# AtomGradient/swift-qwen3-tts

Hardware: AMD Instinct MI355X
Metric: codec_tokens_per_s (higher is better)
Workload: dtype bf16

## Files before the change

### include/q3tts.h

```cpp
#ifndef Q3TTS_H
#define Q3TTS_H

#include <stddef.h>
#include <stdint.h>

#ifdef __cplusplus
extern "C" {
#endif

#define Q3TTS_ABI_VERSION 4

typedef struct q3tts_model q3tts_model;

typedef enum {
    Q3TTS_OK = 0,
    Q3TTS_ERR_MODEL_NOT_INITIALIZED = 1,
    Q3TTS_ERR_GENERATION_FAILED = 2,
    Q3TTS_ERR_INVALID_INPUT = 3,
    Q3TTS_ERR_AUDIO_DECODING_FAILED = 4,
    Q3TTS_ERR_AUDIO_ENCODING_FAILED = 5,
    Q3TTS_ERR_IO = 6,
    Q3TTS_ERR_DEVICE = 7,
    Q3TTS_ERR_CANCELLED = 8,
    Q3TTS_ERR_BUSY = 9
// ... 287 lines not shown
    const uint8_t* active;
    const int32_t* block_table;
    const int32_t* chunk_n_prompt;
    uint16_t* kpool;
    uint16_t* vpool;
    uint16_t* out;
} q3tts_attn_debug;
q3tts_status q3tts_debug_attention(q3tts_model* m, const q3tts_attn_debug* a);

typedef struct {
    int32_t mode, geometry_only;
    int32_t M, K, N;
    int32_t xMB, yMB, ss_ld, y_cols;
    int32_t epi, act_silu, resid, nt_weights, y_tiled;
    int32_t norm, quant, has_bias;
    int32_t ss_count, norm_dim;
    float norm_eps;
    int32_t rider_M, rider_H, rider_MB, rider_ss_count;
    float rider_eps;
    int32_t rode;
    int32_t tall;
    int32_t tall_shape;
    int32_t split, mbw, nw, ch, np, gx, ntw;
    const uint16_t* x;
    const void* W;
    const uint16_t* scales;
    const uint16_t* biases;
    const void* W_up;
    const uint16_t* scales_up;
    const uint16_t* biases_up;
    const uint16_t* bias;
    const uint16_t* norm_w;
    const float* ss_in;
    const uint16_t* rider_h;
    const uint16_t* rider_w;
    const float* rider_ss_in;
    uint16_t* y;
    float* ss_out;
    uint16_t* rider_out;
    float* rider_ss_out;
} q3tts_gemm_debug;
q3tts_status q3tts_debug_gemm(q3tts_model* m, q3tts_gemm_debug* a);

typedef struct {
    int32_t kind, geometry_only, split;
    int32_t B, Tmax, ppf, hist, margin;
// ... 73 lines not shown
```

### swift-qwen3-tts_amd/csrc/debug_env.cc

```cpp
#include <atomic>
#include <cstdlib>
#include <mutex>

#include "kernels.h"

namespace q3 {

namespace {
std::mutex g_mu;
std::atomic<const DebugEnv*> g_env{nullptr};

bool flag(const char* name) { return std::getenv(name) != nullptr; }
int number(const char* name, int dflt) {
    const char* e = std::getenv(name);
    return e && *e ? std::atoi(e) : dflt;
}

const DebugEnv* read_env() {
    DebugEnv* d = new DebugEnv{};
    d->gemm_no_row_split = flag("Q3TTS_GEMM_NO_ROW_SPLIT");
    d->gemm_one_pair = flag("Q3TTS_GEMM_ONE_PAIR");
    d->no_tall_gemm = flag("Q3TTS_NO_TALL_GEMM");
    d->tall_shape = number("Q3TTS_TALL_SHAPE", 0);
    d->chunk_qsplit = number("Q3TTS_CHUNK_QSPLIT", 0);
    d->conv_no_pw = flag("Q3TTS_CONV_NO_PW");
    d->nt_off = std::getenv("Q3TTS_NT") && number("Q3TTS_NT", 1) == 0;
    d->serial_jobs = number("Q3TTS_SERIAL_JOBS", 0) != 0;
    d->fail_back_half = number("Q3TTS_TEST_FAIL_BACK_HALF", 0) != 0;
    d->no_prefix_cache = number("Q3TTS_NO_PREFIX_CACHE", 0) != 0;
    return d;
}
}

const DebugEnv& debug_env() {
    const DebugEnv* e = g_env.load(std::memory_order_acquire);
    if (!e) {
        std::lock_guard<std::mutex> lk(g_mu);
        e = g_env.load(std::memory_order_acquire);
        if (!e) {
            e = read_env();
            g_env.store(e, std::memory_order_release);
        }
    }
    return *e;
// ... 9 lines not shown
```

### swift-qwen3-tts_amd/csrc/engine_debug.cc

```cpp
#include "engine_stream.h"

#include "frontend.h"

namespace q3 {

void Engine::debug_frontend_stage(const float* audio, int64_t n_samples, const char* stage, float* out, int64_t cap, int* T, int* C) {
    Q3_CHECK(fe_ != nullptr, 1, "Model not initialized: Speech tokenizer encoder not available");
    Q3_CHECK(audio && n_samples > 0 && stage, 3, "Invalid input: empty audio or stage name");
    const float* a = upload_audio(audio, n_samples);
    StageCapture cap_s;
    cap_s.name = stage;
    static const char* kSpeaker[] = {"mel", "h0", "h1", "h2", "h3", "mfa", "pooled"};
    bool is_spk = false;
    for (const char* s : kSpeaker) is_spk = is_spk || cap_s.name == s;
    if (is_spk) {
        Q3_CHECK(m_->has_speaker_encoder, 1, "Model not initialized: Speaker encoder not available for this model");
        spk_f32_.grow(size_t(m_->cfg.talker.hidden_size));
        fe_->speaker_embedding(a, n_samples, spk_f32_, &cap_s);
    } else {
        Q3_CHECK(m_->has_codec_encoder, 1, "Model not initialized: Speech tokenizer encoder not available");
        const int Tq = fe_->encoded_frames(n_samples);
        ref_codes_dev_.grow(size_t(16) * Tq);
        fe_->encode(a, n_samples, ref_codes_dev_, &cap_s);
    }
// ... 262 lines not shown
    Q3_HIP(hipMemset(ot, 0xff, size_t(Mp) * odim * 2));
    AttnArgs at{};
    at.qkv = qkv; at.ld = ld; at.qn_w = w; at.kn_w = w + kHeadDim; at.eps = d.eps;
    at.rope_cos = rope; at.rope_sin = rope + tab;
    at.kpool = kp; at.vpool = vp;
    at.block_table = bt; at.max_pages = d.max_pages; at.kv_len = kv_len; at.active = d.active ? (const uint8_t*)act : nullptr;
    at.out = ot; at.outMB = Mp / 16; at.n_heads = d.n_heads; at.n_kv = d.n_kv; at.B = B;
    at.scale = d.scale;
    at.fixed_len = d.fixed_len; at.identity_pages = d.identity_pages ? 1 : 0;
    at.chunk = d.chunk; at.chunk_n_prompt = d.chunk_n_prompt ? n_prompt : nullptr; at.chunk_r_base = d.chunk_r_base;
    at.nt_kv = d.nt_kv ? 1 : 0;
    launch_attn_decode(at, st_);
    Q3_HIP(hipGetLastError());
    launch_untile_rows(ot, Mp / 16, ol, odim, rows, odim, st_);
    Q3_HIP(hipStreamSynchronize(st_));
    Q3_HIP(hipMemcpy(d.out, ol, size_t(rows) * odim * 2, hipMemcpyDeviceToHost));
    Q3_HIP(hipMemcpy(d.kpool, kp, pool * 2, hipMemcpyDeviceToHost));
    Q3_HIP(hipMemcpy(d.vpool, vp, pool * 2, hipMemcpyDeviceToHost));
}

void Engine::debug_gemm_check(q3tts_gemm_debug& d, GemmArgs& ga, NormRowsArgs& na) {
    static const uint16_t dummy16 = 0;
    static const uint32_t dummy32 = 0;
    d.rode = d.tall = d.tall_shape = d.split = d.mbw = d.nw = d.ch = d.np = d.gx = d.ntw = 0;
    Q3_CHECK(d.mode == 0 || d.mode == 1, 3, "debug_gemm: unknown mode");
    const bool rider = d.mode == 1 || d.rider_M > 0;
    if (rider) {
        Q3_CHECK(d.rider_M >= 1 && d.rider_MB >= 1 && d.rider_MB <= 64 && d.rider_M <= 16 * d.rider_MB, 3, "debug_gemm: rider rows out of range");
        Q3_CHECK(d.rider_H >= 128 && d.rider_H <= 4096 && d.rider_H % 128 == 0, 3, "debug_gemm: rider_H must be a multiple of 128 up to 4096");
        Q3_CHECK(d.geometry_only || (d.rider_h && d.rider_w && d.rider_out), 3, "debug_gemm: null rider argument");
        if (d.rider_ss_in) Q3_CHECK(d.rider_ss_count >= 1 && d.rider_ss_count <= 256, 3, "debug_gemm: at most 256 partial sums of squares per rider row");
        na.hMB = na.outMB = d.rider_MB; na.eps = d.rider_eps; na.M = d.rider_M; na.H = d.rider_H;
        na.ss_count = d.rider_ss_in ? d.rider_ss_count : 0; na.ss_ld = 16 * d.rider_MB;
    }
    if (d.mode == 1) return;
    Q3_CHECK(d.epi == 0 || d.epi == 2 || d.epi == 3, 3, "debug_gemm: unknown epilogue");
    Q3_CHECK(d.M >= 1 && d.M <= 1024, 3, "debug_gemm: M out of range");
    Q3_CHECK(d.K >= 128 && d.K <= 8192 && d.K % 128 == 0, 3, "debug_gemm: K must be a multiple of 128 up to 8192");
    Q3_CHECK(d.N >= 8 && d.N <= 65536 && d.N % (d.epi == 2 ? 8 : 16) == 0, 3, "debug_gemm: N must be a multiple of 16 (epi 2: of 8)");
    const int Mp = int(align_up(size_t(d.M), 16));
    const bool tiled = d.epi != 0 || d.y_tiled;
    Q3_CHECK(d.xMB <= 64 && 16 * d.xMB >= Mp && d.yMB <= 64 && 16 * d.yMB >= Mp && d.ss_ld >= Mp && d.ss_ld <= 4096, 3,
             "debug_gemm: allocation smaller than the padded batch");
    Q3_CHECK(d.y_cols >= d.N && d.y_cols <= d.N + 1024 && d.y_cols % (tiled ? 128 : 8) == 0, 3, "debug_gemm: y_cols");
    Q3_CHECK(d.epi != 2 || (!d.has_bias && !d.act_silu), 3, "debug_gemm: the gate/up epilogue takes no bias or activation");
    Q3_CHECK(d.epi == 0 || !d.act_silu, 3, "debug_gemm: act_silu belongs to epi 0");
    Q3_CHECK(d.epi == 3 || (!d.resid && !d.ss_out), 3, "debug_gemm: resid / ss_out belong to epi 3");
    if (d.norm) Q3_CHECK(d.ss_count >= 1 && d.ss_count <= 4096 && d.norm_dim >= 1, 3, "debug_gemm: norm prologue sizes");
    if (!d.geometry_only) {
        Q3_CHECK(d.x && d.W && d.y, 3, "debug_gemm: null argument");
        Q3_CHECK((d.epi == 2) == (d.W_up != nullptr), 3, "debug_gemm: W_up goes with epi 2");
        Q3_CHECK((d.quant != 0) == (d.scales != nullptr) && (d.quant != 0) == (d.biases != nullptr), 3, "debug_gemm: scales / biases go with quant");
        if (d.epi == 2) Q3_CHECK((d.quant != 0) == (d.scales_up != nullptr) && (d.quant != 0) == (d.biases_up != nullptr), 3, "debug_gemm: scales / biases go with quant");
        Q3_CHECK((d.has_bias != 0) == (d.bias != nullptr), 3, "debug_gemm: bias goes with has_bias");
        Q3_CHECK((d.norm != 0) == (d.norm_w != nullptr) && (d.norm != 0) == (d.ss_in != nullptr), 3, "debug_gemm: norm_w / ss_in go with norm");
    }
    ga.Wsb = d.quant ? &dummy32 : nullptr;
    ga.xMB = d.xMB; ga.M = d.M; ga.Mpad = Mp; ga.N = d.N; ga.K = d.K; ga.epi = d.epi;
    ga.ldy = d.y_cols; ga.y_tiled = d.y_tiled ? 1 : 0; ga.yMB = d.yMB;
    ga.bias = d.has_bias ? &dummy16 : nullptr;
    ga.act_silu = d.act_silu ? 1 : 0;
    ga.norm_w = d.norm ? &dummy16 : nullptr;
    ga.ss_count = d.norm ? d.ss_count : 0; ga.ss_ld = d.ss_ld; ga.norm_dim = d.norm_dim; ga.norm_eps = d.norm_eps;
    ga.nt_weights = d.nt_weights ? 1 : 0; ga.resid = d.resid ? 1 : 0;
    const SkinnyGeom g = skinny_geometry(ga);
    d.tall = g.tall ? 1 : 0;
    if (g.tall) {
        d.tall_shape = gemm_tall_shape(ga);
    } else {
        Q3_CHECK(g.mbw >= 1 && g.mbw <= 4, 3, "debug_gemm: more than 4 row blocks per workgroup");
        d.split = g.split; d.mbw = g.mbw; d.nw = g.nw; d.ch = g.ch; d.np = g.np; d.gx = g.gx; d.ntw = g.ntw ? 1 : 0;
    }
    if (rider) d.rode = gemm_norm_rows_rides(ga, na) ? 1 : 0;
}

namespace {
void host_tile(const uint16_t* src, std::vector<uint16_t>& dst, int rows, int cols) {
    dst.resize(size_t(rows) * cols);
    for (int m = 0; m < rows; ++m)
        for (int k = 0; k < cols; k += 8) std::memcpy(&dst[act_tiled_offset(m, k, rows / 16)], src + size_t(m) * cols + k, 16);
}
void host_untile(const std::vector<uint16_t>& src, uint16_t* dst, int rows, int cols) {
    for (int m = 0; m < rows; ++m)
        for (int k = 0; k < cols; k += 8) std::memcpy(dst + size_t(m) * cols + k, &src[act_tiled_offset(m, k, rows / 16)], 16);
}
}

void Engine::debug_gemm(q3tts_gemm_debug& d) {
    GemmArgs ga{};
    NormRowsArgs na{};
    debug_gemm_check(d, ga, na);
    DevBuf<uint16_t> dx, dy, dbias, dnw, dsrc, dsc, dbi, rh, rw, rout;
    DevBuf<uint8_t> dWt;
    DevBuf<uint32_t> dWq, dsb;
// ... 321 lines not shown
```

### swift-qwen3-tts_amd/csrc/kernels.h

```cpp
#pragma once
#include <hip/hip_runtime.h>

#include <cstdint>

namespace q3 {

struct DebugEnv {
    bool gemm_no_row_split;
    bool gemm_one_pair;
    bool no_tall_gemm;
    int tall_shape;
    int chunk_qsplit;
    bool conv_no_pw;
    bool nt_off;
    bool serial_jobs;
    bool fail_back_half;
    bool no_prefix_cache;
};
const DebugEnv& debug_env();
void debug_env_reload();

constexpr int kPageTokens = 64;
constexpr int kHeadDim = 128;

struct NormRowsArgs {
    const uint16_t* h;
    int hMB;
    const uint16_t* w;
    float eps;
    uint16_t* out;
    int outMB;
    float* ss_out;
// ... 10 lines not shown
    int xMB;
    int M, Mpad, N, K;
    int epi;
    uint16_t* y;
    int ldy;
    int y_tiled, yMB;
    const uint16_t* bias;
    int act_silu;
    const uint16_t* norm_w;
    const float* ss_in;
    int ss_count, ss_ld, norm_dim;
    float norm_eps;
    int nt_weights;
    int resid;
    float* ss_out;
};
void launch_gemm_skinny(const GemmArgs& a, hipStream_t st);
struct SkinnyGeom {
    bool tall;
    int split, mbw;
    int nw, ch, np;
    int gx;
    bool ntw;
};
SkinnyGeom skinny_geometry(const GemmArgs& a);
bool launch_gemm_skinny_with_norm_rows(const GemmArgs& a, const NormRowsArgs& n, hipStream_t st);
bool gemm_norm_rows_rides(const GemmArgs& a, const NormRowsArgs& n);
bool launch_gemm_tall(const GemmArgs& a, hipStream_t st);
bool gemm_tall_takes(const GemmArgs& a);
int gemm_tall_shape(const GemmArgs& a);


struct AttnArgs {
    const uint16_t* qkv;
    int ld;
    const uint16_t* qn_w;
    const uint16_t* kn_w;
    float eps;
    const uint16_t* rope_cos;
    const uint16_t* rope_sin;
    uint16_t* kpool;
    uint16_t* vpool;
    const int32_t* block_table;
    int max_pages;
    const int32_t* kv_len;
    const uint8_t* active;
// ... 166 lines not shown
```

### swift-qwen3-tts_amd/csrc/kernels/gemm_body.inc

```
__device__ __forceinline__ f32x4 mfma16(const uint4& a, const uint4& b, f32x4 c) {
    bf16x8 av, bv;
    __builtin_memcpy(&av, &a, 16);
    __builtin_memcpy(&bv, &b, 16);
    return __builtin_amdgcn_mfma_f32_16x16x32_bf16(av, bv, c, 0, 0, 0);
}

__device__ __forceinline__ float silu_f(float v) { return v / (1.0f + __expf(-v)); }

__device__ __forceinline__ uint4 norm8(const uint4& hx, const uint4& wx, float rstd) {
    const uint32_t hw[4] = {hx.x, hx.y, hx.z, hx.w}, ww[4] = {wx.x, wx.y, wx.z, wx.w};
    uint32_t o[4];
#pragma unroll
    for (int j = 0; j < 4; ++j) {
        const float n0 = rbf(lo_bf(hw[j]) * rstd), n1 = rbf(hi_bf(hw[j]) * rstd);
        o[j] = pack_bf(n0 * lo_bf(ww[j]), n1 * hi_bf(ww[j]));
    }
    return make_uint4(o[0], o[1], o[2], o[3]);
}

__device__ __forceinline__ void dequant_chunk(const uint4& qw, uint32_t sb, uint4 (&out)[4]) {
    const float sc = lo_bf(sb), bi = hi_bf(sb);
    const uint32_t w[4] = {qw.x, qw.y, qw.z, qw.w};
#pragma unroll
    for (int i = 0; i < 4; ++i) {
        uint32_t o[4];
#pragma unroll
        for (int j = 0; j < 4; ++j) {
            const float q0 = (float)((w[i] >> (8 * j)) & 15u), q1 = (float)((w[i] >> (8 * j + 4)) & 15u);
            o[j] = pack_bf(__fadd_rn(__fmul_rn(q0, sc), bi), __fadd_rn(__fmul_rn(q1, sc), bi));
        }
        out[i] = make_uint4(o[0], o[1], o[2], o[3]);
    }
}

template <int MB, int EPI, int NW, int CH, bool NORM, bool QUANT, int NP = 1, bool NTW = false>
__device__ __forceinline__ void gemm_skinny_body(const GemmArgs& a, const int tile, const int mb0) {
    constexpr int NT = NP;
    constexpr int NR = 1;
    const int n_tiles = (EPI == 2) ? (a.N >> 3) : (a.N >> 4);
    __shared__ float red[NW][NR][MB][4][64];
    __shared__ __attribute__((aligned(16))) uint16_t ys[MB][16][16];
    __shared__ float rstd_s[NORM ? 16 * MB : 1];
    __shared__ float ssp_s[NORM ? 8 : 1][NORM ? 16 * MB : 1];

    const int lane = threadIdx.x & 63;
    const int wave = threadIdx.x >> 6;
    const int KC = a.K >> 7;

    f32x4 acc[NT][MB];
#pragma unroll
    for (int t = 0; t < NT; ++t)
#pragma unroll
        for (int mb = 0; mb < MB; ++mb) acc[t][mb] = f32x4{0.f, 0.f, 0.f, 0.f};

    const uint4* Wt = reinterpret_cast<const uint4*>(a.W);
    const uint4* Xt = reinterpret_cast<const uint4*>(a.x);

    constexpr int kSsIter = NORM ? (16 * MB * 8 + NW * 64 - 1) / (NW * 64) : 1;
    float sst[kSsIter][16];
    if constexpr (NORM) {
        const int rows = 16 * MB;
#pragma unroll
        for (int it = 0; it < kSsIter; ++it) {
            const int idx = (threadIdx.x + it * NW * 64) % (rows * 8);
            const int row = idx % rows, part = idx / rows;
            const float* sp = a.ss_in + 16 * mb0 + row;
#pragma unroll
            for (int u = 0; u < 16; ++u) {
                const int j = part + 8 * u;
                sst[it][u] = sp[(size_t)(j < a.ss_count ? j : 0) * a.ss_ld];
            }
        }
        __builtin_amdgcn_sched_barrier(0);
    }

    constexpr int CHR = CH > 0 ? CH : 1;
    constexpr int WL = QUANT ? 1 : 4;
    uint4 wf[CHR][NT][WL];
    uint32_t wsb[CHR][NT];
    auto load_w = [&](int c, int kc) {
#pragma unroll
        for (int t = 0; t < NT; ++t) {
            const int tt = tile * NT + t;
            const size_t blk = (size_t)(tt < n_tiles ? tt : n_tiles - 1) * KC + kc;
            if constexpr (QUANT) {
                wf[c][t][0] = ld16<NTW>(Wt + blk * 64 + lane);
                wsb[c][t] = a.Wsb[blk * 64 + lane];
            } else {
                const uint4* wp = Wt + blk * 256 + lane;
#pragma unroll
                for (int i = 0; i < 4; ++i) wf[c][t][i] = ld16<NTW>(wp + i * 64);
            }
        }
    };

    constexpr int kWRegs = CH * NT * (QUANT ? 5 : 16);
    constexpr int kRoom = (((MB == 1 && !NORM) ? 200 : 176) - kWRegs) / (MB * 16);
    constexpr int kCap = (MB == 1 && !NORM) ? 6 : 3;
    constexpr int XG0 = (CH == 0) ? 0 : (kRoom < 1 ? 1 : (kRoom > kCap ? (CH < kCap ? CH : kCap) : (kRoom < CH ? kRoom : CH)));
    constexpr int XG = (MB == 2 && NORM && CH == 2 && NT == 1 && EPI == 0) ? 1 : XG0;
    uint4 xr[XG > 0 ? XG : 1][MB][4];
    uint4 nwr[(NORM && XG > 0) ? XG : 1][4];
#pragma unroll
    for (int ph = 0; ph < 2; ++ph) {
        if (ph == 1) __builtin_amdgcn_sched_barrier(0);
        if ((ph == 0) != NORM) {
    if constexpr (CH > 0) {
#pragma unroll
            for (int c = 0; c < CH; ++c) {
                const int kl = wave + c * NW;
                load_w(c, kl < KC ? kl : 0);
            }
        }
        } else {
    if constexpr (XG > 0) {
#pragma unroll
        for (int c = 0; c < XG; ++c) {
            const int kl = wave + c * NW;
            const int kc = kl < KC ? kl : 0;
            if constexpr (NORM) {
                const uint4* np = reinterpret_cast<const uint4*>(a.norm_w + kc * 128 + 32 * (lane >> 4));
#pragma unroll
                for (int i = 0; i < 4; ++i) nwr[c][i] = np[i];
            }
#pragma unroll
            for (int mb = 0; mb < MB; ++mb) {
                const uint4* xp = Xt + ((size_t)(kc * a.xMB + mb0 + mb) * 4) * 64 + lane;
#pragma unroll
                for (int i = 0; i < 4; ++i) xr[c][mb][i] = xp[i * 64];
            }
        }
    }
        }
    }
// ... 13 lines not shown
        for (int it = 0; it < kSsIter; ++it) {
            const int idx = threadIdx.x + it * NW * 64;
            if (idx < rows * 8) {
                const int row = idx % rows, part = idx / rows;
                float s = 0.f;
#pragma unroll
                for (int u = 0; u < 16; ++u)
                    if (part + 8 * u < a.ss_count) s += sst[it][u];
                for (int j = part + 128; j < a.ss_count; j += 8) s += a.ss_in[(size_t)j * a.ss_ld + 16 * mb0 + row];
                ssp_s[part][row] = s;
            }
        }
        __syncthreads();
        if (threadIdx.x < rows) {
            float s = 0.f;
#pragma unroll
            for (int p = 0; p < 8; ++p) s += ssp_s[p][threadIdx.x];
            rstd_s[threadIdx.x] = 1.0f / sqrtf(s / (float)a.norm_dim + a.norm_eps);
        }
        __syncthreads();
#pragma unroll
        for (int mb = 0; mb < MB; ++mb) rstd[mb] = rstd_s[16 * mb + (lane & 15)];
    }

    auto chunk = [&](int kc, int c, const uint4 (*xpre)[4], const uint4* nwpre) {
        uint4 w[NT][4];
#pragma unroll
        for (int t = 0; t < NT; ++t) {
            if constexpr (QUANT) {
                dequant_chunk(wf[c][t][0], wsb[c][t], w[t]);
            } else {
#pragma unroll
                for (int i = 0; i < 4; ++i) w[t][i] = wf[c][t][i];
            }
        }
        uint4 nw[4];
        if constexpr (NORM) {
            if (nwpre) {
#pragma unroll
                for (int i = 0; i < 4; ++i) nw[i] = nwpre[i];
            } else {
                const uint4* np = reinterpret_cast<const uint4*>(a.norm_w + kc * 128 + 32 * (lane >> 4));
#pragma unroll
                for (int i = 0; i < 4; ++i) nw[i] = np[i];
            }
        }
#pragma unroll
        for (int mb = 0; mb < MB; ++mb) {
            uint4 xf[4];
            if (xpre) {
#pragma unroll
                for (int i = 0; i < 4; ++i) xf[i] = xpre[mb][i];
            } else {
                const uint4* xp = Xt + ((size_t)(kc * a.xMB + mb0 + mb) * 4) * 64 + lane;
#pragma unroll
                for (int i = 0; i < 4; ++i) xf[i] = xp[i * 64];
            }
            if constexpr (NORM) {
#pragma unroll
                for (int i = 0; i < 4; ++i) xf[i] = norm8(xf[i], nw[i], rstd[mb]);
            }
#pragma unroll
            for (int t = 0; t < NT; ++t)
#pragma unroll
                for (int i = 0; i < 4; ++i) acc[t][mb] = mfma16(w[t][i], xf[i], acc[t][mb]);
        }
    };
    if constexpr (CH > 0) {
#pragma unroll
        for (int g0 = 0; g0 < CH; g0 += XG) {
            if (g0 > 0) {
#pragma unroll
                for (int c = 0; c < XG; ++c) {
                    if (g0 + c < CH) {
                        const int kl = wave + (g0 + c) * NW;
                        const int kc = kl < KC ? kl : 0;
                        if constexpr (NORM) {
                            const uint4* np = reinterpret_cast<const uint4*>(a.norm_w + kc * 128 + 32 * (lane >> 4));
#pragma unroll
                            for (int i = 0; i < 4; ++i) nwr[c][i] = np[i];
                        }
#pragma unroll
                        for (int mb = 0; mb < MB; ++mb) {
                            const uint4* xp = Xt + ((size_t)(kc * a.xMB + mb0 + mb) * 4) * 64 + lane;
#pragma unroll
                            for (int i = 0; i < 4; ++i) xr[c][mb][i] = xp[i * 64];
                        }
                    }
                }
            }
#pragma unroll
            for (int c = 0; c < XG; ++c) {
                if (g0 + c < CH) {
                    const int kl = wave + (g0 + c) * NW;
                    if (kl < KC) chunk(kl, g0 + c, xr[c], NORM ? nwr[c] : nullptr);
                }
            }
        }
    } else {
        for (int kl = wave; kl < KC; kl += NW) {
            load_w(0, kl);
            chunk(kl, 0, nullptr, nullptr);
        }
    }

#pragma unroll
    for (int pr = 0; pr < NT / NR; ++pr) {
    if (pr > 0) __syncthreads();
#pragma unroll
    for (int t = 0; t < NR; ++t)
#pragma unroll
        for (int mb = 0; mb < MB; ++mb)
#pragma unroll
            for (int q = 0; q < 4; ++q) red[wave][t][mb][q][lane] = acc[pr * NR + t][mb][q];
    __syncthreads();
    const int otile = tile * (NT / NR) + pr;

    if constexpr (EPI == 2) {
        for (int o = threadIdx.x; o < 128 * MB; o += NW * 64) {
            const int mb = o >> 7, rem = o & 127;
            const int b = rem >> 3, f = rem & 7;
            const int lg = (f >> 2) * 16 + b, lu = (2 + (f >> 2)) * 16 + b, q = f & 3;
            float g = 0.f, u = 0.f;
#pragma unroll
            for (int w = 0; w < NW; ++w) {
                g += red[w][0][mb][q][lg];
                u += red[w][0][mb][q][lu];
            }
            ys[mb][b][f] = f2bf(rbf(silu_f(rbf(g))) * rbf(u));
        }
    } else {
    for (int o = threadIdx.x; o < 256 * MB; o += NW * 64) {
        const int mb = o >> 8, rem = o & 255;
        const int b = rem >> 4, f = rem & 15;
        const int src_lane = (f >> 2) * 16 + b, q = f & 3;
        float sum = 0.f;
#pragma unroll
        for (int w = 0; w < NW; ++w) sum += red[w][0][mb][q][src_lane];
        const int n = otile * 16 + f;
        float y = sum;
        if (a.bias && otile < n_tiles) y += bf2f(a.bias[n]);
        uint16_t yb = f2bf(y);
        if (EPI == 0 && a.act_silu) yb = f2bf(silu_f(bf2f(yb)));
        ys[mb][b][f] = yb;
    }
    }
    __syncthreads();
    if constexpr (EPI == 2) {
        for (int o = threadIdx.x; o < 16 * MB; o += NW * 64) {
            const int mb = o >> 4, b = o & 15;
            const int m = 16 * (mb0 + mb) + b;
            if (m < a.M && otile < n_tiles)
                *reinterpret_cast<uint4*>(a.y + act_tiled_offset(m, otile * 8, a.yMB)) = *reinterpret_cast<const uint4*>(&ys[mb][b][0]);
        }
    } else
    for (int o = threadIdx.x; o < 32 * MB; o += NW * 64) {
        const int mb = o >> 5, b = (o >> 1) & 15, p = o & 1;
        const int m = 16 * (mb0 + mb) + b;
        uint4 v = *reinterpret_cast<const uint4*>(&ys[mb][b][8 * p]);
        const int n = otile * 16 + 8 * p;
        if constexpr (EPI == 3) {
            uint16_t* hp = a.y + act_tiled_offset(m, n, a.yMB);
            float ss = 0.f;
            const uint32_t yw[4] = {v.x, v.y, v.z, v.w};
            uint32_t ow[4];
            uint4 hv = hv_pre;
            if constexpr (NT > 1) {
                if (a.resid && m < a.M && otile < n_tiles) hv = *reinterpret_cast<const uint4*>(hp);
            }
            const uint32_t hw[4] = {hv.x, hv.y, hv.z, hv.w};
#pragma unroll
            for (int j = 0; j < 4; ++j) {
                float h0 = lo_bf(yw[j]), h1 = hi_bf(yw[j]);
                if (a.resid) {
                    h0 = rbf(lo_bf(hw[j]) + h0);
                    h1 = rbf(hi_bf(hw[j]) + h1);
                }
                ss += h0 * h0;
                ss += h1 * h1;
                ow[j] = pack_bf(h0, h1);
            }
            const float other = __shfl_xor(ss, 1, 64);
            if (m < a.M && otile < n_tiles) {
                *reinterpret_cast<uint4*>(hp) = make_uint4(ow[0], ow[1], ow[2], ow[3]);
                if (p == 0 && a.ss_out) a.ss_out[(size_t)otile * a.ss_ld + m] = ss + other;
            }
        } else {
            if (m >= a.M || otile >= n_tiles) continue;
            if (a.y_tiled)
                *reinterpret_cast<uint4*>(a.y + act_tiled_offset(m, n, a.yMB)) = v;
            else
                *reinterpret_cast<uint4*>(a.y + (size_t)m * a.ldy + n) = v;
        }
    }
    }
}
```

### swift-qwen3-tts_amd/csrc/kernels/gemm_decode.hip

```cpp
#include "../common.h"
#include "../kernels.h"
#include "row_jobs.h"

namespace q3 {

namespace {

#include "gemm_body.inc"

template <int MB, int EPI, int NW, int CH, bool NORM, bool QUANT, int NP = 1, bool NTW = false>
__global__ __launch_bounds__(NW * 64) void gemm_skinny_kernel(GemmArgs a) {
    __builtin_amdgcn_s_setprio(3);
    gemm_skinny_body<MB, EPI, NW, CH, NORM, QUANT, NP, NTW>(a, blockIdx.x, blockIdx.y * MB);
}

struct GemmSideArgs {
    GemmArgs g;
    NormRowsArgs n;
    int tiles;
};
template <int MB, int CH, bool QUANT>
__global__ __launch_bounds__(512) void gemm_skinny_side_kernel(GemmSideArgs s) {
    __builtin_amdgcn_s_setprio(3);
    if (int(blockIdx.x) >= s.tiles) {
        __shared__ float side_sh[4];
        __shared__ float side_parts[8];
        if (blockIdx.y == 0) norm_row_job(s.n, int(blockIdx.x) - s.tiles, threadIdx.x, side_sh, side_parts);
        return;
    }
    gemm_skinny_body<MB, 0, 8, CH, true, QUANT, 1, false>(s.g, blockIdx.x, blockIdx.y * MB);
}

template <int MB, int EPI, bool NORM, bool QUANT, bool NTW>
void launch_mb(const GemmArgs& a, const SkinnyGeom& g, hipStream_t st) {
    const dim3 grid(g.gx, g.split);
#define Q3_GEMM(NWv, CHv) \
    hipLaunchKernelGGL((gemm_skinny_kernel<MB, EPI, NWv, CHv, NORM, QUANT, 1, NTW>), grid, dim3(NWv * 64), 0, st, a)
    if constexpr (MB == 4 && !NORM && !NTW) {
        if (g.ch == 0 && g.np == 2) { hipLaunchKernelGGL((gemm_skinny_kernel<4, EPI, 8, 0, false, QUANT, 2, false>), grid, dim3(512), 0, st, a); return; }
        if (g.ch == 0 && g.np == 4) { hipLaunchKernelGGL((gemm_skinny_kernel<4, EPI, 8, 0, false, QUANT, 4, false>), grid, dim3(512), 0, st, a); return; }
    }
    if constexpr (EPI == 2 && MB <= 2) {
        if (g.np > 1) {
#define Q3_GEMM_NP(CHv, NPv) hipLaunchKernelGGL((gemm_skinny_kernel<MB, 2, 8, CHv, NORM, QUANT, NPv, NTW>), grid, dim3(512), 0, st, a)
            if (g.ch == 1) { if (g.np == 2) Q3_GEMM_NP(1, 2); else Q3_GEMM_NP(1, 3); }
            else { if (g.np == 2) Q3_GEMM_NP(2, 2); else Q3_GEMM_NP(2, 3); }
#undef Q3_GEMM_NP
            return;
        }
    }
    if (g.nw == 4) {
        Q3_GEMM(4, 1);
    } else {
        switch (g.ch) {
            case 1: Q3_GEMM(8, 1); break;
            case 2: Q3_GEMM(8, 2); break;
            case 3: Q3_GEMM(8, 3); break;
            case 6: Q3_GEMM(8, 6); break;
            default: Q3_GEMM(8, 0); break;
        }
    }
#undef Q3_GEMM
}

template <int EPI, bool NORM, bool QUANT>
void launch_q(const GemmArgs& a, hipStream_t st) {
// ... 45 lines not shown
    while (MBt / split > 4 || MBt % split != 0) ++split;
    g.split = split;
    g.mbw = MBt / split;
    g.ntw = a.nt_weights && g.mbw <= 2;
    const int KC = a.K / 128;
    g.nw = KC <= 4 ? 4 : 8;
    g.ch = (KC + g.nw - 1) / g.nw;
    g.np = 1;
    const int t = a.epi == 2 ? a.N / 8 : a.N / 16;
    g.gx = t;
    bool shaped = false;
    if (g.mbw == 4 && !norm && !g.ntw && !env.gemm_one_pair && g.nw == 8 && t >= 64) {
        g.np = (((t + 3) / 4) * split <= 128) ? 2 : 4;
        g.ch = 0;
        g.gx = (t + g.np - 1) / g.np;
        shaped = true;
    }
    if (!shaped && a.epi == 2 && g.mbw <= 2) {
        const int np = env.gemm_one_pair ? 1 : (t > 512 ? 3 : (t > 256 ? 2 : 1));
        if (g.nw == 8 && (g.ch == 1 || g.ch == 2) && np > 1) {
            g.np = np;
            g.gx = (t + np - 1) / np;
            shaped = true;
        }
    }
    if (!shaped) {
        if (g.nw == 4) g.ch = 1;
        else if (g.ch != 1 && g.ch != 2 && g.ch != 3 && g.ch != 6) g.ch = 0;
    }
    return g;
}

bool gemm_norm_rows_rides(const GemmArgs& a, const NormRowsArgs& n) {
    if (a.epi != 0 || !a.norm_w || a.nt_weights || n.M <= 0 || n.H > 4096) return false;
    if (a.K % 128 != 0 || a.N % 16 != 0) return false;
    const SkinnyGeom g = skinny_geometry(a);
    return !(g.tall || g.nw != 8 || g.np != 1 || (g.ch != 1 && g.ch != 2) || g.mbw < 1 || g.mbw > 2 || g.ntw);
}

bool launch_gemm_skinny_with_norm_rows(const GemmArgs& a, const NormRowsArgs& n, hipStream_t st) {
    if (!gemm_norm_rows_rides(a, n)) return false;
    const SkinnyGeom g = skinny_geometry(a);
    Q3_CHECK(a.ss_in && a.ss_count >= 1 && a.ss_ld >= a.Mpad && a.xMB * 16 >= a.Mpad, 3, "gemm_skinny: norm prologue needs sums of squares");
    const int tiles = g.gx;
    const dim3 grid(tiles + n.M, g.split), block(512);
    const GemmSideArgs s{a, n, tiles};
// ... 6 lines not shown
    if (g.mbw == 1) { if (g.ch == 1) Q3_SIDE(1, 1); else Q3_SIDE(1, 2); }
    else { if (g.ch == 1) Q3_SIDE(2, 1); else Q3_SIDE(2, 2); }
#undef Q3_SIDE
    return true;
}

void launch_gemm_skinny(const GemmArgs& a, hipStream_t st) {
    Q3_CHECK(a.K % 128 == 0 && a.N % (a.epi == 2 ? 8 : 16) == 0, 3, "gemm_skinny: K must be a multiple of 128 and N of 16");
    Q3_CHECK(a.Mpad % 16 == 0 && a.M <= a.Mpad && a.Mpad <= 1024, 3, "gemm_skinny: bad M padding");
    Q3_CHECK(a.xMB * 16 >= a.Mpad, 3, "gemm_skinny: x allocation has fewer row blocks than the batch");
    const bool norm = a.norm_w != nullptr;
    if (a.epi == 3) Q3_CHECK(a.yMB * 16 >= a.Mpad, 3, "gemm_skinny: h allocation has fewer row blocks than the batch");
    if (launch_gemm_tall(a, st)) return;
    if (norm) Q3_CHECK(a.ss_in && a.ss_count >= 1 && a.ss_ld >= a.Mpad, 3, "gemm_skinny: norm prologue needs sums of squares");
    switch (a.epi) {
        case 0: norm ? launch_epi<0, true>(a, st) : launch_epi<0, false>(a, st); break;
        case 2: norm ? launch_epi<2, true>(a, st) : launch_epi<2, false>(a, st); break;
        case 3: norm ? launch_epi<3, true>(a, st) : launch_epi<3, false>(a, st); break;
        default: throw Error(3, "gemm_skinny: unknown epilogue");
    }
}

}
```

### swift-qwen3-tts_amd/qwen3tts/_lib.py

```python
from __future__ import annotations

import ctypes as C
import os

_HERE = os.path.dirname(os.path.abspath(__file__))
LIB_PATH = os.environ.get("Q3TTS_LIB") or os.path.join(_HERE, "libq3tts_hip.so")

u16p = C.POINTER(C.c_uint16)
i32p = C.POINTER(C.c_int32)
f32p = C.POINTER(C.c_float)
u8p = C.POINTER(C.c_uint8)


class LoadOpts(C.Structure):
    _fields_ = [("device", C.c_int32), ("max_batch", C.c_int32), ("max_frames", C.c_int32),
                ("max_prompt", C.c_int32), ("use_graph", C.c_int32), ("weights_from_broadcast", C.c_int32),
                ("n_streams", C.c_int32), ("codec_overlap_cus", C.c_int32), ("codec_fp32", C.c_int32),
                ("output_sample_rate", C.c_int32), ("speed", C.c_float), ("request_speeds", C.c_int32)]


class LoadOptsEx(C.Structure):
    _fields_ = [("base", LoadOpts), ("pitch", C.c_float)]


# ... 79 lines not shown

ERR_CANCELLED, ERR_BUSY = 8, 9


class AttnDebug(C.Structure):
    _fields_ = [("n_heads", C.c_int32), ("n_kv", C.c_int32), ("B", C.c_int32), ("eps", C.c_float), ("scale", C.c_float),
                ("max_pages", C.c_int32), ("fixed_len", C.c_int32), ("identity_pages", C.c_int32), ("chunk", C.c_int32),
                ("chunk_r_base", C.c_int32), ("nt_kv", C.c_int32), ("n_pos", C.c_int32), ("n_pages", C.c_int32),
                ("qkv", u16p), ("qn_w", u16p), ("kn_w", u16p), ("rope_cos", u16p), ("rope_sin", u16p),
                ("kv_len", i32p), ("active", u8p), ("block_table", i32p), ("chunk_n_prompt", i32p),
                ("kpool", u16p), ("vpool", u16p), ("out", u16p)]


class GemmDebug(C.Structure):
    _fields_ = [("mode", C.c_int32), ("geometry_only", C.c_int32), ("M", C.c_int32), ("K", C.c_int32), ("N", C.c_int32),
                ("xMB", C.c_int32), ("yMB", C.c_int32), ("ss_ld", C.c_int32), ("y_cols", C.c_int32),
                ("epi", C.c_int32), ("act_silu", C.c_int32), ("resid", C.c_int32), ("nt_weights", C.c_int32), ("y_tiled", C.c_int32),
                ("norm", C.c_int32), ("quant", C.c_int32), ("has_bias", C.c_int32), ("ss_count", C.c_int32), ("norm_dim", C.c_int32),
                ("norm_eps", C.c_float),
                ("rider_M", C.c_int32), ("rider_H", C.c_int32), ("rider_MB", C.c_int32), ("rider_ss_count", C.c_int32),
                ("rider_eps", C.c_float),
                ("rode", C.c_int32), ("tall", C.c_int32), ("tall_shape", C.c_int32),
                ("split", C.c_int32), ("mbw", C.c_int32), ("nw", C.c_int32), ("ch", C.c_int32), ("np", C.c_int32), ("gx", C.c_int32),
                ("ntw", C.c_int32),
                ("x", u16p), ("W", C.c_void_p), ("scales", u16p), ("biases", u16p), ("W_up", C.c_void_p), ("scales_up", u16p),
                ("biases_up", u16p), ("bias", u16p), ("norm_w", u16p), ("ss_in", f32p), ("rider_h", u16p), ("rider_w", u16p),
                ("rider_ss_in", f32p),
                ("y", u16p), ("ss_out", f32p), ("rider_out", u16p), ("rider_ss_out", f32p)]


class ConvDebug(C.Structure):
    _fields_ = [("kind", C.c_int32), ("geometry_only", C.c_int32), ("split", C.c_int32),
                ("B", C.c_int32), ("Tmax", C.c_int32), ("ppf", C.c_int32), ("hist", C.c_int32), ("margin", C.c_int32),
                ("Cin", C.c_int32), ("N", C.c_int32), ("K", C.c_int32), ("dil", C.c_int32),
                ("ldx", C.c_int32), ("ldo", C.c_int32), ("ldr", C.c_int32), ("ldx2", C.c_int32),
                ("act", C.c_int32), ("pre_act", C.c_int32), ("shift", C.c_int32), ("reflect", C.c_int32), ("post_C", C.c_int32),
                ("x_f32", C.c_int32), ("res_is_out", C.c_int32),
                ("family", C.c_int32), ("BN", C.c_int32), ("pro", C.c_int32), ("pw_depth", C.c_int32), ("KT", C.c_int32),
                ("X32", C.c_int32), ("CT2", C.c_int32), ("PT", C.c_int32), ("wdb", C.c_int32),
                ("grid_x", C.c_int32), ("grid_y", C.c_int32), ("grid_z", C.c_int32), ("lds_bytes", C.c_int64),
                ("frames", i32p), ("x", C.c_void_p), ("x2", f32p), ("w", f32p), ("w2", f32p), ("bias", f32p), ("bias2", f32p),
                ("scale", f32p), ("snake_alpha", f32p), ("snake_beta", f32p), ("act2_alpha", f32p), ("act2_beta", f32p),
                ("post_alpha", f32p), ("post_beta", f32p), ("res", C.c_void_p),
                ("out", C.c_void_p), ("out2", C.c_void_p), ("pcm", f32p), ("nonfinite", i32p)]


class RowopDebug(C.Structure):
# ... 123 lines not shown
    L.q3tts_tokenizer_free.restype = None
    L.q3tts_tokenizer_encode.argtypes = [vp, C.c_char_p, i32p, C.c_int32, i32p]
    L.q3tts_debug_prepare_inputs.argtypes = [vp, C.POINTER(Request), u16p, C.c_int32, i32p, u16p, C.c_int32,
                                             i32p, u16p]
    L.q3tts_debug_generate_forced.argtypes = [vp, C.POINTER(Request), C.c_int32, C.POINTER(Sampling), i32p,
                                              C.c_int32, u16p, u16p, i32p]
    L.q3tts_debug_sample.argtypes = [vp, u16p, C.c_int32, C.c_int32, C.POINTER(Sampling), u8p, C.c_int32,
                                     C.c_int32, C.c_int32, C.c_uint32, C.c_uint32, i32p]
    L.q3tts_debug_linear.argtypes = [vp, u16p, u16p, u16p, C.c_int32, C.c_int32, C.c_int32, u16p]
    L.q3tts_debug_attention.argtypes = [vp, C.POINTER(AttnDebug)]
    if hasattr(L, "q3tts_debug_gemm"):
        L.q3tts_debug_gemm.argtypes = [vp, C.POINTER(GemmDebug)]
    if hasattr(L, "q3tts_debug_conv"):
        L.q3tts_debug_conv.argtypes = [vp, C.POINTER(ConvDebug)]
    if hasattr(L, "q3tts_debug_rowop"):
        L.q3tts_debug_rowop.argtypes = [vp, C.POINTER(RowopDebug)]
    if hasattr(L, "q3tts_debug_build_decode_codes"):
        L.q3tts_debug_build_decode_codes.argtypes = [vp, i32p, i32p, i32p, i32p, C.c_int32, C.c_int32, C.c_int32, C.c_int32, i32p]
    L.q3tts_debug_codec_stage.argtypes = [vp, i32p, C.c_int32, C.c_char_p, f32p, C.c_int64, i32p, i32p]
    _lib = L
    return L


GEOM_FIELDS = ("rode", "tall", "tall_shape", "split", "mbw", "nw", "ch", "np", "gx", "ntw")


def gemm_geometry(**kw) -> dict:
    a = GemmDebug(geometry_only=1, **kw)
    st = lib().q3tts_debug_gemm(None, C.byref(a))
    if st != 0:
        raise ValueError("q3tts_debug_gemm refused the arguments (status %d): %r" % (st, kw))
    return {f: int(getattr(a, f)) for f in GEOM_FIELDS}


CONV_GEOM_FIELDS = ("family", "BN", "pro", "pw_depth", "KT", "X32", "CT2", "PT", "wdb", "grid_x", "grid_y", "grid_z", "lds_bytes")
CONV_OPERANDS = ("x2", "bias", "bias2", "scale", "snake", "act2", "post", "res", "out", "out2", "w2", "pcm", "nonfinite")


def conv_geometry(frames=None, **kw) -> dict:
    ops = {k: kw.pop(k, False) for k in CONV_OPERANDS}
    a = ConvDebug(geometry_only=1, **kw)
    one = (C.c_float * 4)()
    fp = C.cast(one, f32p)
    a.w = fp
    for name in ("x2", "bias", "bias2", "scale", "w2", "pcm"):
        if ops[name]:
            setattr(a, name, fp)
# ... 22 lines not shown
```

Measured before the change: 10200.

## Add tile-major gate/up GEMM order that overlaps tile epilogues with deferred loads

Adds a tile-major variant of the skinny fused-norm gate/up GEMM that issues weight loads for every chunk of each output tile, defers the last tile's loads until after the norm, and then reduces and writes each tile in turn. Separate reduction and staging buffers per tile let one tile's epilogue overlap the next tile's MFMAs without the per-tile sync. It becomes the default for two specific geometries and can be switched off with an env flag. The cost is more LDS and register pressure. A compile-time wall-clock timeline probe is also added.

```diff
diff --git a/include/q3tts.h b/include/q3tts.h
--- a/include/q3tts.h
+++ b/include/q3tts.h
@@ -333,6 +333,7 @@
     int32_t tall;
     int32_t tall_shape;
     int32_t split, mbw, nw, ch, np, gx, ntw;
+    int32_t tm;
     const uint16_t* x;
     const void* W;
     const uint16_t* scales;
diff --git a/swift-qwen3-tts_amd/csrc/debug_env.cc b/swift-qwen3-tts_amd/csrc/debug_env.cc
--- a/swift-qwen3-tts_amd/csrc/debug_env.cc
+++ b/swift-qwen3-tts_amd/csrc/debug_env.cc
@@ -20,6 +20,7 @@
     DebugEnv* d = new DebugEnv{};
     d->gemm_no_row_split = flag("Q3TTS_GEMM_NO_ROW_SPLIT");
     d->gemm_one_pair = flag("Q3TTS_GEMM_ONE_PAIR");
+    d->gemm_parent_forms = number("Q3TTS_GEMM_PARENT_FORMS", 0) != 0;
     d->no_tall_gemm = flag("Q3TTS_NO_TALL_GEMM");
     d->tall_shape = number("Q3TTS_TALL_SHAPE", 0);
     d->chunk_qsplit = number("Q3TTS_CHUNK_QSPLIT", 0);
diff --git a/swift-qwen3-tts_amd/csrc/engine_debug.cc b/swift-qwen3-tts_amd/csrc/engine_debug.cc
--- a/swift-qwen3-tts_amd/csrc/engine_debug.cc
+++ b/swift-qwen3-tts_amd/csrc/engine_debug.cc
@@ -308,7 +308,7 @@
 void Engine::debug_gemm_check(q3tts_gemm_debug& d, GemmArgs& ga, NormRowsArgs& na) {
     static const uint16_t dummy16 = 0;
     static const uint32_t dummy32 = 0;
-    d.rode = d.tall = d.tall_shape = d.split = d.mbw = d.nw = d.ch = d.np = d.gx = d.ntw = 0;
+    d.rode = d.tall = d.tall_shape = d.split = d.mbw = d.nw = d.ch = d.np = d.gx = d.ntw = d.tm = 0;
     Q3_CHECK(d.mode == 0 || d.mode == 1, 3, "debug_gemm: unknown mode");
     const bool rider = d.mode == 1 || d.rider_M > 0;
     if (rider) {
@@ -355,7 +355,7 @@
         d.tall_shape = gemm_tall_shape(ga);
     } else {
         Q3_CHECK(g.mbw >= 1 && g.mbw <= 4, 3, "debug_gemm: more than 4 row blocks per workgroup");
-        d.split = g.split; d.mbw = g.mbw; d.nw = g.nw; d.ch = g.ch; d.np = g.np; d.gx = g.gx; d.ntw = g.ntw ? 1 : 0;
+        d.split = g.split; d.mbw = g.mbw; d.nw = g.nw; d.ch = g.ch; d.np = g.np; d.gx = g.gx; d.ntw = g.ntw ? 1 : 0; d.tm = g.tm ? 1 : 0;
     }
     if (rider) d.rode = gemm_norm_rows_rides(ga, na) ? 1 : 0;
 }
diff --git a/swift-qwen3-tts_amd/csrc/kernels.h b/swift-qwen3-tts_amd/csrc/kernels.h
--- a/swift-qwen3-tts_amd/csrc/kernels.h
+++ b/swift-qwen3-tts_amd/csrc/kernels.h
@@ -8,6 +8,7 @@
 struct DebugEnv {
     bool gemm_no_row_split;
     bool gemm_one_pair;
+    bool gemm_parent_forms;
     bool no_tall_gemm;
     int tall_shape;
     int chunk_qsplit;
@@ -64,6 +65,7 @@
     int nw, ch, np;
     int gx;
     bool ntw;
+    bool tm;
 };
 SkinnyGeom skinny_geometry(const GemmArgs& a);
 bool launch_gemm_skinny_with_norm_rows(const GemmArgs& a, const NormRowsArgs& n, hipStream_t st);
diff --git a/swift-qwen3-tts_amd/csrc/kernels/gemm_body.inc b/swift-qwen3-tts_amd/csrc/kernels/gemm_body.inc
--- a/swift-qwen3-tts_amd/csrc/kernels/gemm_body.inc
+++ b/swift-qwen3-tts_amd/csrc/kernels/gemm_body.inc
@@ -1,3 +1,34 @@
+#ifdef Q3TTS_GEMM_TIMELINE
+__device__ unsigned long long g_gemm_tl[4][2][8][8];
+#define Q3_TL_BEGIN()                                                                                                       \
+    constexpr int kTlForm = (EPI == 2 && MB == 2 && NW == 8 && CH == 2 && NP == 3 && NTW) ? (TM ? 1 : 0)                    \
+                            : ((EPI == 3 && MB == 1 && NW == 8 && CH == 6 && !NORM && NTW) ? 2                              \
+                               : ((EPI == 0 && MB == 2 && NW == 8 && CH == 2 && NORM && NP == 1 && NTW) ? 3 : -1));         \
+    unsigned long long tl_[8] = {0, 0, 0, 0, 0, 0, 0, 0};                                                                   \
+    Q3_TL(0)
+#define Q3_TL(k)                                   \
+    do {                                           \
+        if constexpr (kTlForm >= 0) {              \
+            __builtin_amdgcn_sched_barrier(0);     \
+            tl_[k] = wall_clock64();               \
+            __builtin_amdgcn_sched_barrier(0);     \
+        }                                          \
+    } while (0)
+#define Q3_TL_END()                                                                                                         \
+    do {                                                                                                                    \
+        if constexpr (kTlForm >= 0) {                                                                                       \
+            const bool tl_last = blockIdx.x == gridDim.x - 1 && blockIdx.y == gridDim.y - 1;                                \
+            if ((tl_last || (blockIdx.x == 0 && blockIdx.y == 0)) && lane == 0) {                                           \
+                _Pragma("unroll") for (int k = 0; k < 8; ++k) g_gemm_tl[kTlForm][tl_last ? 1 : 0][wave][k] = tl_[k];        \
+            }                                                                                                               \
+        }                                                                                                                   \
+    } while (0)
+#else
+#define Q3_TL_BEGIN() ((void)0)
+#define Q3_TL(k) ((void)0)
+#define Q3_TL_END() ((void)0)
+#endif
+
 __device__ __forceinline__ f32x4 mfma16(const uint4& a, const uint4& b, f32x4 c) {
     bf16x8 av, bv;
     __builtin_memcpy(&av, &a, 16);
@@ -33,18 +64,22 @@
     }
 }
 
-template <int MB, int EPI, int NW, int CH, bool NORM, bool QUANT, int NP = 1, bool NTW = false>
+template <int MB, int EPI, int NW, int CH, bool NORM, bool QUANT, int NP = 1, bool NTW = false, bool TM = false>
 __device__ __forceinline__ void gemm_skinny_body(const GemmArgs& a, const int tile, const int mb0) {
     constexpr int NT = NP;
     constexpr int NR = 1;
+    constexpr int NB = TM ? NT : 1;
+    constexpr int kDefer = TM ? NT - 1 : 0;
+    static_assert(!TM || (EPI == 2 && NORM && !QUANT && CH > 0 && NP > 1), "tile-major order is a gate/up form");
     const int n_tiles = (EPI == 2) ? (a.N >> 3) : (a.N >> 4);
-    __shared__ float red[NW][NR][MB][4][64];
-    __shared__ __attribute__((aligned(16))) uint16_t ys[MB][16][16];
+    __shared__ float red[NB][NW][NR][MB][4][64];
+    __shared__ __attribute__((aligned(16))) uint16_t ys[NB][MB][16][16];
     __shared__ float rstd_s[NORM ? 16 * MB : 1];
     __shared__ float ssp_s[NORM ? 8 : 1][NORM ? 16 * MB : 1];
 
     const int lane = threadIdx.x & 63;
     const int wave = threadIdx.x >> 6;
+    Q3_TL_BEGIN();
     const int KC = a.K >> 7;
 
     f32x4 acc[NT][MB];
@@ -78,9 +113,9 @@
     constexpr int WL = QUANT ? 1 : 4;
     uint4 wf[CHR][NT][WL];
     uint32_t wsb[CHR][NT];
-    auto load_w = [&](int c, int kc) {
-#pragma unroll
-        for (int t = 0; t < NT; ++t) {
+    auto load_w = [&](int c, int kc, int t0, int t1) {
+#pragma unroll
+        for (int t = t0; t < t1; ++t) {
             const int tt = tile * NT + t;
             const size_t blk = (size_t)(tt < n_tiles ? tt : n_tiles - 1) * KC + kc;
             if constexpr (QUANT) {
@@ -99,17 +134,26 @@
     constexpr int kCap = (MB == 1 && !NORM) ? 6 : 3;
     constexpr int XG0 = (CH == 0) ? 0 : (kRoom < 1 ? 1 : (kRoom > kCap ? (CH < kCap ? CH : kCap) : (kRoom < CH ? kRoom : CH)));
     constexpr int XG = (MB == 2 && NORM && CH == 2 && NT == 1 && EPI == 0) ? 1 : XG0;
+    static_assert(!TM || XG == CH, "tile-major order keeps every chunk's x fragments in registers");
     uint4 xr[XG > 0 ? XG : 1][MB][4];
     uint4 nwr[(NORM && XG > 0) ? XG : 1][4];
 #pragma unroll
     for (int ph = 0; ph < 2; ++ph) {
         if (ph == 1) __builtin_amdgcn_sched_barrier(0);
         if ((ph == 0) != NORM) {
-    if constexpr (CH > 0) {
+    if constexpr (TM) {
+#pragma unroll
+            for (int t = 0; t < NT - kDefer; ++t)
+#pragma unroll
+                for (int c = 0; c < CH; ++c) {
+                    const int kl = wave + c * NW;
+                    load_w(c, kl < KC ? kl : 0, t, t + 1);
+                }
+    } else if constexpr (CH > 0) {
 #pragma unroll
             for (int c = 0; c < CH; ++c) {
                 const int kl = wave + c * NW;
-                load_w(c, kl < KC ? kl : 0);
+                load_w(c, kl < KC ? kl : 0, 0, NT);
             }
         }
         } else {
@@ -169,6 +213,25 @@
 #pragma unroll
         for (int mb = 0; mb < MB; ++mb) rstd[mb] = rstd_s[16 * mb + (lane & 15)];
     }
+    Q3_TL(1);
+    if constexpr (TM) {
+#pragma unroll
+        for (int c = 0; c < CH; ++c) {
+#pragma unroll
+            for (int mb = 0; mb < MB; ++mb)
+#pragma unroll
+                for (int i = 0; i < 4; ++i) xr[c][mb][i] = norm8(xr[c][mb][i], nwr[c][i], rstd[mb]);
+        }
+        __builtin_amdgcn_sched_barrier(0);
+#pragma unroll
+        for (int t = NT - kDefer; t < NT; ++t)
+#pragma unroll
+            for (int c = 0; c < CH; ++c) {
+                const int kl = wave + c * NW;
+                load_w(c, kl < KC ? kl : 0, t, t + 1);
+            }
+        __builtin_amdgcn_sched_barrier(0);
+    }
 
     auto chunk = [&](int kc, int c, const uint4 (*xpre)[4], const uint4* nwpre) {
         uint4 w[NT][4];
@@ -213,7 +276,8 @@
                 for (int i = 0; i < 4; ++i) acc[t][mb] = mfma16(w[t][i], xf[i], acc[t][mb]);
         }
     };
-    if constexpr (CH > 0) {
+    if constexpr (TM) {
+    } else if constexpr (CH > 0) {
 #pragma unroll
         for (int g0 = 0; g0 < CH; g0 += XG) {
             if (g0 > 0) {
@@ -242,25 +306,43 @@
                     const int kl = wave + (g0 + c) * NW;
                     if (kl < KC) chunk(kl, g0 + c, xr[c], NORM ? nwr[c] : nullptr);
                 }
+                if (g0 + c == 0) Q3_TL(2);
             }
         }
     } else {
         for (int kl = wave; kl < KC; kl += NW) {
-            load_w(0, kl);
+            load_w(0, kl, 0, NT);
             chunk(kl, 0, nullptr, nullptr);
         }
     }
 
+    if constexpr (!TM) Q3_TL(3);
 #pragma unroll
     for (int pr = 0; pr < NT / NR; ++pr) {
-    if (pr > 0) __syncthreads();
+    const int rb = TM ? pr : 0;
+    if constexpr (TM) {
+#pragma unroll
+        for (int c = 0; c < CH; ++c) {
+            if (wave + c * NW < KC) {
+#pragma unroll
+                for (int mb = 0; mb < MB; ++mb)
+#pragma unroll
+                    for (int i = 0; i < 4; ++i) acc[pr][mb] = mfma16(wf[c][pr][i], xr[c][mb][i], acc[pr][mb]);
+            }
+        }
+        if (pr == 0) Q3_TL(2);
+        if (pr == NT - 1) Q3_TL(3);
+    } else {
+        if (pr > 0) __syncthreads();
+    }
 #pragma unroll
     for (int t = 0; t < NR; ++t)
 #pragma unroll
         for (int mb = 0; mb < MB; ++mb)
 #pragma unroll
-            for (int q = 0; q < 4; ++q) red[wave][t][mb][q][lane] = acc[pr * NR + t][mb][q];
+            for (int q = 0; q < 4; ++q) red[rb][wave][t][mb][q][lane] = acc[pr * NR + t][mb][q];
     __syncthreads();
+    if (pr == NT / NR - 1) Q3_TL(4);
     const int otile = tile * (NT / NR) + pr;
 
     if constexpr (EPI == 2) {
@@ -271,10 +353,10 @@
             float g = 0.f, u = 0.f;
 #pragma unroll
             for (int w = 0; w < NW; ++w) {
-                g += red[w][0][mb][q][lg];
-                u += red[w][0][mb][q][lu];
-            }
-            ys[mb][b][f] = f2bf(rbf(silu_f(rbf(g))) * rbf(u));
+                g += red[rb][w][0][mb][q][lg];
+                u += red[rb][w][0][mb][q][lu];
+            }
+            ys[rb][mb][b][f] = f2bf(rbf(silu_f(rbf(g))) * rbf(u));
         }
     } else {
     for (int o = threadIdx.x; o < 256 * MB; o += NW * 64) {
@@ -283,28 +365,30 @@
         const int src_lane = (f >> 2) * 16 + b, q = f & 3;
         float sum = 0.f;
 #pragma unroll
-        for (int w = 0; w < NW; ++w) sum += red[w][0][mb][q][src_lane];
+        for (int w = 0; w < NW; ++w) sum += red[rb][w][0][mb][q][src_lane];
         const int n = otile * 16 + f;
         float y = sum;
         if (a.bias && otile < n_tiles) y += bf2f(a.bias[n]);
         uint16_t yb = f2bf(y);
         if (EPI == 0 && a.act_silu) yb = f2bf(silu_f(bf2f(yb)));
-        ys[mb][b][f] = yb;
+        ys[rb][mb][b][f] = yb;
     }
     }
     __syncthreads();
+    if (pr == 0) Q3_TL(7);
+    if (pr == NT / NR - 1) Q3_TL(5);
     if constexpr (EPI == 2) {
         for (int o = threadIdx.x; o < 16 * MB; o += NW * 64) {
             const int mb = o >> 4, b = o & 15;
             const int m = 16 * (mb0 + mb) + b;
             if (m < a.M && otile < n_tiles)
-                *reinterpret_cast<uint4*>(a.y + act_tiled_offset(m, otile * 8, a.yMB)) = *reinterpret_cast<const uint4*>(&ys[mb][b][0]);
+                *reinterpret_cast<uint4*>(a.y + act_tiled_offset(m, otile * 8, a.yMB)) = *reinterpret_cast<const uint4*>(&ys[rb][mb][b][0]);
         }
     } else
     for (int o = threadIdx.x; o < 32 * MB; o += NW * 64) {
         const int mb = o >> 5, b = (o >> 1) & 15, p = o & 1;
         const int m = 16 * (mb0 + mb) + b;
-        uint4 v = *reinterpret_cast<const uint4*>(&ys[mb][b][8 * p]);
+        uint4 v = *reinterpret_cast<const uint4*>(&ys[rb][mb][b][8 * p]);
         const int n = otile * 16 + 8 * p;
         if constexpr (EPI == 3) {
             uint16_t* hp = a.y + act_tiled_offset(m, n, a.yMB);
@@ -341,4 +425,6 @@
         }
     }
     }
+    Q3_TL(6);
+    Q3_TL_END();
 }
diff --git a/swift-qwen3-tts_amd/csrc/kernels/gemm_decode.hip b/swift-qwen3-tts_amd/csrc/kernels/gemm_decode.hip
--- a/swift-qwen3-tts_amd/csrc/kernels/gemm_decode.hip
+++ b/swift-qwen3-tts_amd/csrc/kernels/gemm_decode.hip
@@ -8,10 +8,10 @@
 
 #include "gemm_body.inc"
 
-template <int MB, int EPI, int NW, int CH, bool NORM, bool QUANT, int NP = 1, bool NTW = false>
+template <int MB, int EPI, int NW, int CH, bool NORM, bool QUANT, int NP = 1, bool NTW = false, bool TM = false>
 __global__ __launch_bounds__(NW * 64) void gemm_skinny_kernel(GemmArgs a) {
     __builtin_amdgcn_s_setprio(3);
-    gemm_skinny_body<MB, EPI, NW, CH, NORM, QUANT, NP, NTW>(a, blockIdx.x, blockIdx.y * MB);
+    gemm_skinny_body<MB, EPI, NW, CH, NORM, QUANT, NP, NTW, TM>(a, blockIdx.x, blockIdx.y * MB);
 }
 
 struct GemmSideArgs {
@@ -42,6 +42,13 @@
     }
     if constexpr (EPI == 2 && MB <= 2) {
         if (g.np > 1) {
+            if constexpr (MB == 2 && NORM && !QUANT) {
+                if constexpr (NTW) {
+                    if (g.tm) { hipLaunchKernelGGL((gemm_skinny_kernel<2, 2, 8, 2, true, false, 3, true, true>), grid, dim3(512), 0, st, a); return; }
+                } else {
+                    if (g.tm) { hipLaunchKernelGGL((gemm_skinny_kernel<2, 2, 8, 1, true, false, 2, false, true>), grid, dim3(512), 0, st, a); return; }
+                }
+            }
 #define Q3_GEMM_NP(CHv, NPv) hipLaunchKernelGGL((gemm_skinny_kernel<MB, 2, 8, CHv, NORM, QUANT, NPv, NTW>), grid, dim3(512), 0, st, a)
             if (g.ch == 1) { if (g.np == 2) Q3_GEMM_NP(1, 2); else Q3_GEMM_NP(1, 3); }
             else { if (g.np == 2) Q3_GEMM_NP(2, 2); else Q3_GEMM_NP(2, 3); }
@@ -133,6 +140,7 @@
             g.np = np;
             g.gx = (t + np - 1) / np;
             shaped = true;
+            g.tm = !env.gemm_parent_forms && g.mbw == 2 && norm && !a.Wsb && ((g.ntw && g.ch == 2 && np == 3) || (!g.ntw && g.ch == 1 && np == 2));
         }
     }
     if (!shaped) {
@@ -185,3 +193,10 @@
 }
 
 }
+
+#ifdef Q3TTS_GEMM_TIMELINE
+extern "C" int q3tts_debug_gemm_timeline(unsigned long long* out) {
+    if (hipDeviceSynchronize() != hipSuccess) return 7;
+    return hipMemcpyFromSymbol(out, HIP_SYMBOL(q3::g_gemm_tl), sizeof(q3::g_gemm_tl)) == hipSuccess ? 0 : 7;
+}
+#endif
diff --git a/swift-qwen3-tts_amd/qwen3tts/_lib.py b/swift-qwen3-tts_amd/qwen3tts/_lib.py
--- a/swift-qwen3-tts_amd/qwen3tts/_lib.py
+++ b/swift-qwen3-tts_amd/qwen3tts/_lib.py
@@ -125,7 +125,7 @@
                 ("rider_eps", C.c_float),
                 ("rode", C.c_int32), ("tall", C.c_int32), ("tall_shape", C.c_int32),
                 ("split", C.c_int32), ("mbw", C.c_int32), ("nw", C.c_int32), ("ch", C.c_int32), ("np", C.c_int32), ("gx", C.c_int32),
-                ("ntw", C.c_int32),
+                ("ntw", C.c_int32), ("tm", C.c_int32),
                 ("x", u16p), ("W", C.c_void_p), ("scales", u16p), ("biases", u16p), ("W_up", C.c_void_p), ("scales_up", u16p),
                 ("biases_up", u16p), ("bias", u16p), ("norm_w", u16p), ("ss_in", f32p), ("rider_h", u16p), ("rider_w", u16p),
                 ("rider_ss_in", f32p),
@@ -295,7 +295,7 @@
     return L
 
 
-GEOM_FIELDS = ("rode", "tall", "tall_shape", "split", "mbw", "nw", "ch", "np", "gx", "ntw")
+GEOM_FIELDS = ("rode", "tall", "tall_shape", "split", "mbw", "nw", "ch", "np", "gx", "ntw", "tm")
 
 
 def gemm_geometry(**kw) -> dict:
```

Result: no change. 10480 (median of 6 runs) (+2.7%).
